# DankerMu/SHUD-up

Hardware: AMD Instinct MI355X
Metric: element-flux-updates/sec (RHS evals × NumEle) at 1/2/4/8 GPUs; %HBM roofline (higher is better)
Workload: dtype f64

## Files before the change

shud-up_amd/csrc/shud_dev.h:

```cpp
#pragma once
#include <hip/hip_runtime.h>
#include <stdint.h>

namespace shud {

constexpr int kWarnSlots = 64, kWarnStride = 16;
struct DevErr {
    uint32_t flags;
    int32_t first_index[8];
    unsigned long long n_warn;
    unsigned long long *warn;
};

struct DevMesh {
    int num_ele;
    const int *nabr, *eflags;
    const double *area, *z_surf, *z_bottom, *depression, *edge, *dist2nabor, *dist2edge, *avg_rough, *rough;
    const double *aq, *macD, *macKsatH, *vAreaF, *KsatH, *KsatV, *infKsatV, *hAreaF, *macKsatV;
    const double *ThetaS, *ThetaR, *Beta, *infD, *Sy, *RzD, *VegFrac, *ImpAF;
    const double *net_prep, *pot_evap, *pot_tran, *etp, *lai, *fu_surf, *fu_sub, *prcp;
    double *e_ic[2], *u_satn[2];
    const double *ugw_stale;
    const double *eybc, *eqbc, *rybc, *rqbc;
    const int *seg_off, *seg_riv;
    const double *seg_len, *seg_cwr;
    double *qseg_surf, *qseg_sub;
    const int *riv_down, *riv_bc;
    const double *riv_len, *riv_slope, *riv_d2down, *riv_avg_rough, *riv_depth, *riv_bw, *riv_bankslope;
    const double *riv_ksath, *riv_bedthick;
    const int *up_off, *up_idx;
    const int *rseg_off, *rseg_pos;
    DevErr *err;
};

enum ClassField {
    CF_macD, CF_macKsatH, CF_vAreaF, CF_KsatH, CF_KsatV, CF_infKsatV, CF_hAreaF, CF_macKsatV, CF_ThetaS,
    CF_ThetaR, CF_Beta, CF_infD, CF_Sy, CF_RzD, CF_VegFrac, CF_ImpAF, CF_depression, CF_rough,
    CF_NPRIMARY,
    CF_fcmr = CF_NPRIMARY,
    CF_dTh,
    CF_ex1, CF_ex2,
    CF_pj,
    CF_omh,
    CF_kmax,
    CF_ekA, CF_ekB,
    CF_r_fcmr, CF_r_dTh, CF_r_infD, CF_r_Sy,
    CF_COUNT
};
constexpr bool cf_stored(int f) { return f != CF_hAreaF && f != CF_macKsatV && f != CF_Beta && f != CF_ImpAF; }
constexpr int cf_pos(int f) {
    int q = 0;
    for (int g = 0; g < f; g++) q += cf_stored(g) ? 1 : 0;
    return cf_stored(f) ? q : -1;
}
template <int F> struct CfPos {
    static_assert(F >= 0 && F < CF_COUNT && cf_stored(F), "field not in the class record");
    static constexpr int v = cf_pos(F);
};
constexpr int CF_NSTORED = cf_pos(CF_COUNT - 1) + 1;
constexpr int CF_STRIDE = CF_NSTORED | 1;
constexpr double kCdivBmin = 0x1p-20, kCdivBmax = 0x1p20;
inline bool cdiv_divisor_ok(double b) {
    const double a = b < 0 ? -b : b;
    return b == 0. || !(a < 1e308) || (a >= kCdivBmin && a <= kCdivBmax);
}
constexpr int kLdsClassMax = 128;
constexpr int kShareTile = 256;
constexpr int kLspN = 5;
constexpr size_t kLspLdsMax = 23296;
constexpr size_t lsp_lds_bytes(int ntab) { return (size_t)(ntab + kLspN * kShareTile) * 8 + kShareTile * 4; }
#ifndef SHUD_PT_COMPACT
#define SHUD_PT_COMPACT 1
#endif
constexpr int kPowTabLogDoubles = SHUD_PT_COMPACT ? 2 * 128 + 64 : 4 * 256;
constexpr int kPowTabDoubles = kPowTabLogDoubles + 2 * 128;
constexpr int kLdsClassMaxBig = 560;
constexpr int kHybMax = 4;

struct DevPacked {
    const double *ctab;
    int ncls;
    int pt_off, ntab;
    const double *hv;
    int nh, hs;
    int hnb;
    signed char hslot1[CF_NPRIMARY];
    const double2 *zz;
    const int4 *meta;
    const double2 *ged;
    const double *area;
    int *seg_first;
    const double2 *sg_lc;
    const int *sg_r;
    const double2 *rrec;
    double2 *qseg2;
    double2 *s_np;
    double2 *s_tl;
    double2 *s_fu;
    double2 *cs[2];
    const double2 *rv;
    const int4 *rv_u;
    int riv_sb;
    double *qdown;
    int nqd;
    int qd_pm, qd_pm_fold;
    int lds_big;
};

struct DevDiag {
    double *qele_surf, *qele_sub, *qele_surf_tot, *qele_sub_tot, *q_infil, *q_exfil, *q_recharge;
    double *q_es, *q_eu, *q_eg, *q_tu, *q_tg, *q_eta, *e_ic, *u_satn, *i_beta, *eff_kh;
    double *qe2r_surf, *qe2r_sub, *qriv_down, *qriv_up, *qriv_surf, *qriv_sub;
    double *q_lake_surf, *q_lake_sub, *q_lake_rivin, *q_lake_evap, *q_lake_prcp, *lake_toparea;
};

struct DevLake {
    int nl;
    int y_off;
    const int *lake_of;
    double *bank_qs, *bank_qg;
    const int *bathy_off;
    const double *bathy_y, *bathy_a;
    const int *ele_off, *ele_idx;
    const int *bank_off, *bank_pos;
    const int *rin_off, *rin_idx;
};

struct YView {
    const double *y;
    const double *gele;
    const double *griv;
    int n_own, n_own_riv;
#ifdef __HIPCC__
    __device__ __forceinline__ double sf(int i) const { return i < n_own ? y[i] : gele[3 * (i - n_own)]; }
    __device__ __forceinline__ double us(int i) const { return i < n_own ? y[n_own + i] : gele[3 * (i - n_own) + 1]; }
    __device__ __forceinline__ double gw(int i) const { return i < n_own ? y[2 * n_own + i] : gele[3 * (i - n_own) + 2]; }
    __device__ __forceinline__ double riv(int r) const { return r < n_own_riv ? y[3 * n_own + r] : griv[r - n_own_riv]; }
    template <bool GH> __device__ __forceinline__ double sf_(int i) const { return GH ? sf(i) : y[i]; }
    template <bool GH> __device__ __forceinline__ double us_(int i) const { return GH ? us(i) : y[n_own + i]; }
    template <bool GH> __device__ __forceinline__ double gw_(int i) const { return GH ? gw(i) : y[2 * n_own + i]; }
    template <bool GH> __device__ __forceinline__ double riv_(int r) const { return GH ? riv(r) : y[3 * n_own + r]; }
#endif
};

void launch_element_kernel(const DevMesh &m, const YView &Y, double *dy, int n_compute, int cur, int cur_e,
                           int mode, bool open, bool diag, const DevDiag &dg, hipStream_t s);
bool launch_element_kernel_packed(const DevMesh &m, const DevPacked &p, const YView &Y, double *dy, int i0, int i1,
                                  int cur, int mode, bool open, bool diag, bool fu_unit, const DevDiag &dg,
                                  hipStream_t s, const DevLake *lake = nullptr, bool interior = false,
                                  bool with_qd = false);
// ... 23 lines not shown
```

shud-up_amd/csrc/shud_ele_packed.hip:

```cpp
#include <hip/hip_runtime.h>
#include <stdint.h>
#include <stdlib.h>

#include "shud_dev.h"
#include "shud_physics.h"

namespace shud {

typedef double v2d __attribute__((ext_vector_type(2)));
typedef int v4i __attribute__((ext_vector_type(4)));
template <class T>
__device__ __forceinline__ T ldnt(const T *p) { return __builtin_nontemporal_load(p); }
__device__ __forceinline__ double2 ldnt2(const double2 *p) {
    const v2d v = __builtin_nontemporal_load((const v2d *)p);
    return make_double2(v.x, v.y);
}
__device__ __forceinline__ int4 ldnt4(const int4 *p) {
    const v4i v = __builtin_nontemporal_load((const v4i *)p);
    return make_int4(v.x, v.y, v.z, v.w);
}
__device__ __forceinline__ void stnt2(double2 *p, double a, double b) {
    v2d v;
    v.x = a;
    v.y = b;
    __builtin_nontemporal_store(v, (v2d *)p);
}
template <class T>
__device__ __forceinline__ const T *at(const T *b, uint32_t off) { return (const T *)((const char *)b + off); }
template <class T>
__device__ __forceinline__ T *atw(T *b, uint32_t off) { return (T *)((char *)b + off); }

__device__ __forceinline__ bool nan_or_inf(double x) { return __builtin_isfpclass(x, 0x0003 | 0x0004 | 0x0200); }
__device__ __forceinline__ bool bad_nonneg(double x) {
    return __builtin_isfpclass(x, 0x0003 | 0x0004 | 0x0008 | 0x0010 | 0x0200);
}

__device__ __forceinline__ const double *riv_y_at(const YView &Y, int r) {
    return r < Y.n_own_riv ? Y.y + 3 * (size_t)Y.n_own + r : Y.griv + (r - Y.n_own_riv);
}

__device__ __forceinline__ int cf_ibc(int cf) { return (int)(int8_t)(cf & 0xff); }
__device__ __forceinline__ int cf_iss(int cf) { return (cf >> 8) & 3; }
__device__ __forceinline__ int cf_nseg(int cf) { return (cf >> 10) & 63; }
__device__ __forceinline__ int cf_class(int cf) { return (int)(((unsigned)cf >> 16) & 0x7fffu); }

template <int MODE>
__device__ __forceinline__ double ugw_pk(const DevMesh &m, double ygw_raw, int ibc, int j) {
    if (ibc == 0) return MODE == 0 ? ygw_raw : rmax(0.0, ygw_raw);
    if (ibc > 0) return m.eybc[ibc];
    return m.ugw_stale[j];
}

constexpr int LDS_CLS_MAX = kLdsClassMax;
constexpr int CF_LDS_STRIDE = CF_STRIDE;

constexpr int kEleWaves = 5;
constexpr int kEleWavesSh = 7;
constexpr bool kShareOn(bool lct, bool gh, bool lake, int hyb, bool diag) {
    return lct && !gh && !lake && hyb == 0 && !diag;
}
constexpr int kEleWavesOf(bool lct, int lspk, bool gh, bool lake, int hyb, bool diag, bool fu1, bool open) {
    return (kShareOn(lct, gh, lake, hyb, diag) && lspk) ? (fu1 ? kEleWavesSh : 6)
           : (kShareOn(lct, gh, lake, hyb, diag) && !open) ? 6 : kEleWaves;
}
constexpr int kEleBS = 256;
static_assert(kEleBS == kShareTile, "edge sharing pairs elements within one workgroup's tile");
static_assert(2 * kEleBS <= kPowTabDoubles, "edge-sharing slots fit the pow tables' LDS region");
constexpr uint64_t kShareVoid = 0x7ff0000000000001ull;
struct OwnRec {
    int4 mt;
    double2 zz, snp, stl, fu, csv;
    double ysf, yus, ygw;
    int sfl;
};
template <bool FU1, bool GH>
__device__ __forceinline__ OwnRec load_own(const DevPacked &p, const YView &Y, int i, int cur) {
    const int nown = Y.n_own;
    const uint32_t o16 = (uint32_t)i << 4, o8 = (uint32_t)i << 3;
    OwnRec o;
    o.mt = *at(p.meta, o16);
    o.zz = *at(p.zz, o16);
    o.ysf = GH ? Y.sf(i) : *at(Y.y, o8);
    o.yus = GH ? Y.us(i) : *at(Y.y + nown, o8);
    o.ygw = GH ? Y.gw(i) : *at(Y.y + 2 * (size_t)nown, o8);
    o.snp = ldnt2(at(p.s_np, o16));
    o.stl = ldnt2(at(p.s_tl, o16));
    if (FU1) { o.fu.x = 1.0; o.fu.y = 1.0; } else o.fu = ldnt2(at(p.s_fu, o16));
    o.csv = ldnt2(at(p.cs[cur], o16));
    o.sfl = *at(p.seg_first, (uint32_t)i << 2);
    return o;
}

constexpr int kTabBatch = 8;
template <int BS>
__device__ __forceinline__ void tab_issue(const DevPacked &p, double (&tv)[kTabBatch]) {
    const int nt2 = (p.ntab + 1) >> 1;
#pragma unroll
    for (int k = 0; k < kTabBatch / 2; k++) {
        const int t = (int)threadIdx.x + k * BS;
        const double2 v = t < nt2 ? ((const double2 *)p.ctab)[t] : make_double2(0., 0.);
        tv[2 * k] = v.x;
        tv[2 * k + 1] = v.y;
    }
}
template <int BS>
__device__ __forceinline__ void tab_store(const DevPacked &p, const double (&tv)[kTabBatch], double *lct) {
    const int nt2 = (p.ntab + 1) >> 1;
#pragma unroll
    for (int k = 0; k < kTabBatch / 2; k++) {
        const int t = (int)threadIdx.x + k * BS;
        if (t < nt2) ((double2 *)lct)[t] = make_double2(tv[2 * k], tv[2 * k + 1]);
    }
    for (int t = (int)threadIdx.x + kTabBatch / 2 * BS; t < nt2; t += BS)
        ((double2 *)lct)[t] = ((const double2 *)p.ctab)[t];
}
__device__ __forceinline__ int tile_of(int per8, int b) { return (b & 7) * per8 + (b >> 3); }
__device__ __forceinline__ int tile_of(int per8) { return tile_of(per8, (int)blockIdx.x); }

struct HaloWait;
template <int MODE, bool HALO>
__device__ __forceinline__ void qd_pre(const DevMesh &m, const DevPacked &p, const YView &Y, int r, int n_int,
                                       const HaloWait *hw);
__device__ __forceinline__ int qd_split(int b, int nb_q, int q0, int *e) {
    if (nb_q && b >= q0 && b < q0 + nb_q) return b - q0;
    *e = b < q0 ? b : b - nb_q;
    return -1;
}

template <int MODE, bool OPEN, bool DIAG, bool FU1, bool LCT, bool LAKE, bool GH, int HYB = 0, int LSP = 0, int BS = 256>
__device__ __forceinline__ void ele_body(const DevMesh &m, const DevPacked &p, const YView &Y, double *__restrict__ dy,
                                         int i, int cur, const DevDiag &dg, const DevLake &lk, const double *lct,
                                         const OwnRec &own);

template <int MODE, bool OPEN, bool DIAG, bool FU1, bool LCT, bool LAKE, bool GH, int HYB = 0, int LSPK = 0>
__global__ void __launch_bounds__(kEleBS, kEleWavesOf(LCT, LSPK, GH, LAKE, HYB, DIAG, FU1, OPEN))
shud_ele_kernel_packed(DevMesh m, DevPacked p, YView Y, double *__restrict__ dy, int i0, int n_compute, int cur,
                       DevDiag dg, DevLake lk, int per8, int nb_q, int q0) {
    extern __shared__ double lct[];
    int eb = (int)blockIdx.x;
    const int qb = qd_split((int)blockIdx.x, nb_q, q0, &eb);
    if (qb >= 0) {
        const int r = qb * kEleBS + (int)threadIdx.x;
        if (r < p.nqd) qd_pre<MODE, false>(m, p, Y, r, 0, nullptr);
        return;
    }
    const int i = i0 + tile_of(per8, eb) * kEleBS + (int)threadIdx.x;
    const bool act = i < n_compute;
    double tv[kTabBatch];
    if (LCT) tab_issue<kEleBS>(p, tv);
    OwnRec own;
    if (act) own = load_own<FU1, GH>(p, Y, i, cur);
    if (LCT) {
        tab_store<kEleBS>(p, tv, lct);
        __syncthreads();
    }
    if (act) ele_body<MODE, OPEN, DIAG, FU1, LCT, LAKE, GH, HYB, LCT ? LSPK : 0>(m, p, Y, dy, i, cur, dg, lk, lct, own);
}

template <int MODE, bool OPEN, bool DIAG, bool FU1, bool GH>
__global__ void __launch_bounds__(1024, 4)
shud_ele_kernel_packed_big(DevMesh m, DevPacked p, YView Y, double *__restrict__ dy, int i0, int n_compute, int cur,
                           DevDiag dg, DevLake lk, int per8) {
    extern __shared__ double lct[];
    const int i = i0 + tile_of(per8) * 1024 + (int)threadIdx.x;
    const bool act = i < n_compute;
    double tv[kTabBatch];
    tab_issue<1024>(p, tv);
    OwnRec own;
    if (act) own = load_own<FU1, GH>(p, Y, i, cur);
    tab_store<1024>(p, tv, lct);
    __syncthreads();
    if (act) ele_body<MODE, OPEN, DIAG, FU1, true, false, GH, 0, 0, 1024>(m, p, Y, dy, i, cur, dg, lk, lct, own);
}

__device__ __forceinline__ void halo_wait(const DevMesh &m, const HaloWait &hw, int i) {
    if (hw.epoch == 0) return;
    bool late = false;
    if (__lane_id() == 0) {
        const unsigned long long t0 = wall_clock64();
        while (__hip_atomic_load(hw.flag, __ATOMIC_RELAXED, __HIP_MEMORY_SCOPE_AGENT) < hw.epoch) {
            __builtin_amdgcn_s_sleep(8);
            if (wall_clock64() - t0 > hw.timeout) { late = true; break; }
        }
    }
    __builtin_amdgcn_fence(__ATOMIC_ACQUIRE, "agent");
    asm volatile("s_waitcnt vmcnt(0)" ::: "memory");
    report_w(m.err, late, 0x80u, 7, i);
}
template <int MODE, bool OPEN, bool FU1, int LSPK = 0>
__global__ void __launch_bounds__(256, kEleWaves)
shud_ele_kernel_packed_fold(DevMesh m, DevPacked p, YView Y, double *__restrict__ dy, int n_int, int n_all, int cur,
                            DevDiag dg, int per8, int nb_int, HaloWait hw, int nb_q, int q0) {
    extern __shared__ double lct[];
    const DevLake lk{};
    int b = (int)blockIdx.x;
    const int qb = qd_split((int)blockIdx.x, nb_q, q0, &b);
    if (qb >= 0) {
        const int r = qb * 256 + (int)threadIdx.x;
        qd_pre<MODE, true>(m, p, Y, r < p.nqd ? r : -1, n_int, &hw);
        return;
    }
    if (b < nb_int) {
        const int i = tile_of(per8, b) * 256 + (int)threadIdx.x;
        const bool act = i < n_int;
        double tv[kTabBatch];
        tab_issue<256>(p, tv);
        OwnRec own;
        if (act) own = load_own<FU1, false>(p, Y, i, cur);
        tab_store<256>(p, tv, lct);
        __syncthreads();
        if (act) ele_body<MODE, OPEN, false, FU1, true, false, false, 0, LSPK>(m, p, Y, dy, i, cur, dg, lk, lct, own);
        return;
    }
    const int i = n_int + (b - nb_int) * 256 + (int)threadIdx.x;
    const bool act = i < n_all;
    double tv[kTabBatch];
    tab_issue<256>(p, tv);
    halo_wait(m, hw, act ? i : n_int);
    OwnRec own;
    if (act) own = load_own<FU1, true>(p, Y, i, cur);
    tab_store<256>(p, tv, lct);
    __syncthreads();
    if (act) ele_body<MODE, OPEN, false, FU1, true, false, true, 0, LSPK>(m, p, Y, dy, i, cur, dg, lk, lct, own);
}
__global__ void shud_halo_flag_kernel(unsigned long long *flag, unsigned long long epoch) {
    if (threadIdx.x == 0) {
        __builtin_amdgcn_fence(__ATOMIC_RELEASE, "agent");
        asm volatile("s_waitcnt vmcnt(0)" ::: "memory");
        __hip_atomic_store(flag, epoch, __ATOMIC_RELAXED, __HIP_MEMORY_SCOPE_AGENT);
    }
}
__global__ void shud_spin_kernel(unsigned long long ticks) {
    if (threadIdx.x == 0) {
        const unsigned long long t0 = wall_clock64();
        while (wall_clock64() - t0 < ticks) __builtin_amdgcn_s_sleep(4);
    }
}
__global__ void shud_copy_f64_kernel(double *__restrict__ dst, const double *__restrict__ src, size_t n) {
    for (size_t k = blockIdx.x * (size_t)blockDim.x + threadIdx.x; k < n; k += (size_t)gridDim.x * blockDim.x)
        dst[k] = src[k];
}

__device__ __forceinline__ double hsel(const double (&v)[4], int k) {
    return k == 1 ? v[0] : k == 2 ? v[1] : k == 3 ? v[2] : v[3];
}
__device__ __forceinline__ void hload(const DevPacked &p, int i, double (&v)[4]) {
    v[1] = 0.; v[2] = 0.; v[3] = 0.;
    if (p.hs == 1) {
        v[0] = p.hv[i];
        return;
    }
    const double2 a = *(const double2 *)(p.hv + (size_t)p.hs * i);
    v[0] = a.x; v[1] = a.y;
    if (p.hs == 4) {
        const double2 b = *(const double2 *)(p.hv + (size_t)p.hs * i + 2);
        v[2] = b.x; v[3] = b.y;
    }
}

template <int MODE, bool OPEN, bool DIAG, bool FU1, bool LCT, bool LAKE, bool GH, int HYB, int LSP, int BS>
__device__ __forceinline__ void ele_body(const DevMesh &m, const DevPacked &p, const YView &Y, double *__restrict__ dy,
                                         int i, int cur, const DevDiag &dg, const DevLake &lk, const double *lct,
                                         const OwnRec &own) {
    const int NEl = m.num_ele;
    const int nown = Y.n_own;
    const uint32_t o16 = (uint32_t)i << 4, o8 = (uint32_t)i << 3;
    (void)o16;
    const int4 mt = own.mt;
    const double2 zz = own.zz;
    const double ysf_raw = own.ysf, yus_raw = own.yus, ygw_raw = own.ygw;
    const int cf = mt.w;
    const int cid = cf_class(cf), ibc = cf_ibc(cf);
    const bool is_lake = LAKE && cf < 0;
    const double2 snp = own.snp, stl = own.stl;
    const double etp = stl.y;
    const double2 fu = own.fu;
    const double2 csv = own.csv;
#define REPORT(c, bit, slot, cnt) report_w(m.err, (c), (bit), (slot), i, (cnt))
#define REPORT_ET(c, bit) (rep |= (c) ? (uint32_t)(bit) : 0u)
#define CL(f) (LCT ? lct[cid * CF_LDS_STRIDE + CfPos<CF_##f>::v] : p.ctab[cid * CF_STRIDE + CfPos<CF_##f>::v])
#define CDIV(a, F) cdiv(a, CL(F), CL(r_##F))
    double hvo[4] = {0., 0., 0., 0.};
    if (HYB == 1) hvo[0] = p.hv[i];
    else if (HYB == 2) hload(p, i, hvo);
#define CLH(f) ((HYB && p.hslot1[CF_##f]) ? (HYB == 1 ? hvo[0] : hsel(hvo, p.hslot1[CF_##f])) : CL(f))
#define CDIV_SY(a) ((HYB && p.hslot1[CF_Sy]) ? (a) / (HYB == 1 ? hvo[0] : hsel(hvo, p.hslot1[CF_Sy])) : CDIV(a, Sy))

    double usf = ysf_raw, uus = yus_raw;
    if (MODE == 1) { usf = (usf >= 0.) ? usf : 0.; uus = (uus >= 0.) ? uus : 0.; }
    const double ugw = ugw_pk<MODE>(m, ygw_raw, ibc, i);
    const double zs = zz.x, zb = zz.y;
    const double aq = zs - zb;

    double ekh, deficit, theta, satn, satkr;
    if (is_lake) {
        ekh = CLH(KsatH); deficit = 0.; satn = 1.; theta = CL(ThetaS); satkr = 1.0;
    } else {
        ekh = eff_kh(ugw, aq, CLH(macD), CLH(macKsatH), CLH(vAreaF), CLH(KsatH));
        REPORT(ekh < 0. || ekh > 1e9, 0x02u, 1, false);
        deficit = aq - ugw;
        const double ThS = CL(ThetaS), ThR = CL(ThetaR);
        if (deficit <= 0.) { deficit = 0.; satn = 1.; theta = ThS; }
        else { theta = uus / deficit * ThS; satn = CDIV(theta - ThR, dTh); }
        if (satn > 0.99) { satn = 1.0; satkr = 1.0; theta = ThS; }
        else if (satn <= K_ZERO) { satn = 0.; satkr = 0.; theta = ThR; }
        else {
// ... 42 lines not shown
            report_w(m.err, rep & 0x10u, 0x10u, 4, i, true);
        }
        if (DIAG) { dg.q_es[i] = Es; dg.q_eu[i] = Eu; dg.q_eg[i] = Eg; dg.q_tu[i] = Tu; dg.q_tg[i] = Tg;
                    dg.q_eta[i] = eta; dg.i_beta[i] = ibeta; }
    }
    stnt2(atw(p.cs[cur ^ 1], o16), satn, eic);

    double qi = 0., qex = 0., qr = 0.;
    if (!is_lake) {
        const double kmax = CL(kmax);
        const double av = usf + snp.x;
        if (ugw + uus > aq || deficit < uus) {
            qex = fabs(ugw + uus - aq) / aq * kmax;
        } else if (av > 0. && deficit > infD) {
            const double grad = 1. + CDIV(av, infD);
            double ek;
            if (av > kmax) ek = CL(ekA) + CL(ekB) * satn;
            else if (av > infK) ek = satkr * infK * CL(omh) + CL(ekB) * satn;
            else ek = satkr * infK * CL(omh);
            qi = rmin(av, rmax(0., grad * ek));
        }
        const double KV = CLH(KsatV);
        if (!(ugw > aq - infD && uus < deficit)) {
            double grad = 0.;
            if (theta > ThR && !(uus <= K_EPSILON)) {
                grad = CDIV(theta - ThR, fcmr);
                grad = rmax(grad, 0.);
            }
            if (!(infK <= 0. || KV <= 0.)) {
                const double ku = infK * satkr;
                qr = grad * ((ku * KV) * (deficit + ugw) / (deficit * KV + ugw * ku));
            }
        }
    }
    const double q_infil = qi * fu_surf, q_exfil = qex * fu_surf;
    const double q_rech = is_lake ? 0. : qr * fu_sub;

    const double dsf_head = snp.x - q_infil + q_exfil;
    const double dgw_head = q_rech - q_exfil;
    typedef __attribute__((address_space(3))) volatile double lds_vd;
    lds_vd *lsp = LSP ? (lds_vd *)(lct + p.ntab) + threadIdx.x : nullptr;
    typedef __attribute__((address_space(3))) volatile int lds_vi;
    lds_vi *lspi = LSP ? (lds_vi *)(lct + p.ntab + kLspN * kEleBS) + threadIdx.x : nullptr;
    if (LSP) {
        lsp[0] = Es; lsp[kEleBS] = Eg; lsp[2 * kEleBS] = Tg; lsp[3 * kEleBS] = dsf_head; lsp[4 * kEleBS] = dgw_head;
        lspi[0] = cf;
    }
    if (i < nown) __builtin_nontemporal_store(is_lake ? 0. : CDIV_SY(q_infil - q_rech - Eu - Tu), atw(dy + nown, o8));

    const double dep = CLH(depression), rgh = CLH(rough);
    double qe2r_surf = 0., qe2r_sub = 0.;
    if (nseg) {
        const double isf_seg = rmax(0., usf - q_infil + q_exfil);
        for (int k = sfirst, k1 = k + nseg; k < k1; k++) {
            const uint32_t k16 = (uint32_t)k << 4;
            const double2 lc = *at(p.sg_lc, k16);
            const int rr = *at(p.sg_r, (uint32_t)k << 2);
            const double2 dk = p.rrec[2 * (size_t)rr], rx = p.rrec[2 * (size_t)rr + 1];
            const int rbc = __builtin_bit_cast(int2, rx.y).x;
            const double bt = rx.x;
            double yr = GH ? Y.riv(rr) : *at(Y.y + 3 * (size_t)nown, (uint32_t)rr << 3);
            if (MODE == 1) yr = (yr >= 0.) ? yr : 0.;
            if (rbc > 0) yr = m.rybc[rbc];
            const double rdep = dk.x, L = lc.x;
            const double qs = weir_jtoi(zs, isf_seg, zs - rdep, yr, zs + 0.0, lc.y, L, dep);
            const double qg = r2e_gw(yr, zs - rdep, ugw, zb, ekh, dk.y, L, bt) * fu_sub;
            *atw(p.qseg2, k16) = make_double2(qs, qg);
            qe2r_surf += -qs;
            qe2r_sub += -qg;
        }
    }
    if (DIAG) {
        dg.q_infil[i] = q_infil; dg.q_exfil[i] = q_exfil; dg.q_recharge[i] = q_rech;
        dg.e_ic[i] = eic; dg.u_satn[i] = satn; dg.eff_kh[i] = ekh;
        dg.qe2r_surf[i] = qe2r_surf; dg.qe2r_sub[i] = qe2r_sub;
    }
    if (i >= nown) return;

    bool nan_q = false;
    const double isf = usf < 0. ? 0. : usf;
    const double area = ldnt(at(p.area, o8));
    const int n_edges = is_lake ? 0 : 3;
    constexpr bool SH = kShareOn(LCT, GH, LAKE, HYB, DIAG) && LSP != 0 && BS == kEleBS;
    auto edge = [&](int j, double &qsf, double &q, uint32_t &sh) __attribute__((always_inline)) {
        const int nb = j == 0 ? mt.x : j == 1 ? mt.y : mt.z;
        const int nc = nb >= 0 ? nb : i;
        const uint32_t n16 = (uint32_t)nc << 4, n8 = (uint32_t)nc << 3;
        const double2 g = ldnt2(at(p.ged, o16 + (uint32_t)j * ((uint32_t)NEl << 4)));
        const double2 nzz = *at(p.zz, n16);
        const int ncf = *at((const int *)p.meta + 3, n16);
        const double nsf_raw = GH ? Y.sf(nc) : *at(Y.y, n8);
        const double ngw_raw = GH ? Y.gw(nc) : *at(Y.y + 2 * (size_t)nown, n8);
        const double B = g.x, d2n = g.y;
        const Recip R2 = recip_nr(d2n);
        qsf = 0.; q = 0.; sh = 0u;
        const double dep_e = SH ? (double)((lds_vd *)lct)[cid * CF_LDS_STRIDE + CfPos<CF_depression>::v] : dep;
        const double rgh_e = SH ? (double)((lds_vd *)lct)[cid * CF_LDS_STRIDE + CfPos<CF_rough>::v] : rgh;
        const int cn = cf_class(ncf);
#define CN(f) (LCT ? lct[cn * CF_LDS_STRIDE + CfPos<CF_##f>::v] : p.ctab[cn * CF_STRIDE + CfPos<CF_##f>::v])
        double hvn[4] = {0., 0., 0., 0.};
        if (HYB == 1 && p.hnb) hvn[0] = p.hv[nc];
        else if (HYB == 2 && p.hnb) hload(p, nc, hvn);
#define CNH(f) ((HYB && p.hslot1[CF_##f]) ? (HYB == 1 ? hvn[0] : hsel(hvn, p.hslot1[CF_##f])) : CN(f))
        if (LAKE && nb >= 0 && ncf < 0) {
            const int l = lk.lake_of[nb];
            const double zl = lk.bathy_y[lk.bathy_off[l]];
            const double yl = Y.y[lk.y_off + l];
            const double nsf = yl < 0. ? 0. : yl;
            qsf = weir_jtoi(zl, nsf, zs, isf, zs, 0.6, B, 0.01);
            const double dhg = (ugw + zb) - (yl + zl);
            if (dhg > 0. && ugw <= 0.02) q = 0.;
            else if (dhg < 0. && yl <= 0.02) q = 0.;
            else {
                const double ymg = (rmax(ugw, 0.) + rmax(yl, 0.)) * .5;
                const double grad = div_nr(dhg, R2);
                const double kmean = 0.5 * (ekh + CNH(KsatH));
                q = kmean * grad * ymg * B;
            }
            lk.bank_qs[(size_t)j * NEl + i] = qsf;
            lk.bank_qg[(size_t)j * NEl + i] = q;
        } else if (nb >= 0) {
            double nsf = nsf_raw;
            if (MODE == 1) nsf = (nsf >= 0.) ? nsf : 0.;
            nsf = nsf < 0. ? 0. : nsf;
            const double zsn = nzz.x;
            const double dh = (isf + zs) - (nsf + zsn);
            [[maybe_unused]] const bool dh_nz = dh != 0., dh_ok = dh == dh;
            double ym = ((isf + zs) > (nsf + zsn)) ? ((isf > dep_e) ? isf : 0.) : ((nsf > dep_e) ? nsf : 0.);
            ym = rmin(ym, K_MAXYSURF);
            bool mu = false;
            if (ym > 0.) {
                const double s = div_nr(dh, R2);
                if (s > 0 && isf <= 0) qsf = 0.;
                else if (s < 0 && nsf <= 0) qsf = 0.;
                else { qsf = manning(ym * B, 0.5 * (rgh_e + CNH(rough)), ym, s); mu = true; }
            }
            const double ugn = ugw_pk<MODE>(m, ngw_raw, cf_ibc(ncf), nb);
            const double zbn = nzz.y;
            const double dhg = (ugw + zb) - (ugn + zbn);
            [[maybe_unused]] const bool dhg_nz = dhg != 0., dhg_ok = dhg == dhg;
            bool zq = true;
            if (dhg > 0. && ugw <= 0.02) q = 0.;
            else if (dhg < 0. && ugn <= 0.02) q = 0.;
            else {
                const double ekn = eff_kh(ugn, zsn - zbn, CNH(macD), CNH(macKsatH), CNH(vAreaF), CNH(KsatH));
                const double ymg = (rmax(ugw, 0.) + rmax(ugn, 0.)) * .5;
                const double grad = div_nr(dhg, R2);
                const double kmean = 0.5 * (ekh + ekn);
                q = kmean * grad * ymg * B;
                zq = false;
            }
            if constexpr (SH) sh = (mu && dh_nz ? 1u : 0u) | (!zq && dhg_nz ? 2u : 0u) | (dh_ok && dhg_ok ? 4u : 0u);
        } else if (OPEN) {
            const double d2e = m.dist2edge[j * NEl + i];
            if (isf > dep_e) {
                const double s = isf / d2e * 0.5;
                if (s > 0.) qsf = sqrt(s) * cbrt(isf * isf * isf * isf * isf) * B / rgh_e;
            }
            if (ugw > dep_e * 10.) {
                const double grad = ugw / d2e * 0.5;
                if (grad > 0.) q = ekh * grad;
            }
        }
#undef CN
#undef CNH
    };
    double sumsurf = qe2r_surf, sumsub = qe2r_sub;
    auto add = [&](int j, double qsf, double q) __attribute__((always_inline)) {
        const double qsb = q * fu_sub;
        if (MODE == 0) nan_q |= nan_or_inf(qsf) || nan_or_inf(qsb);
        sumsurf += qsf;
        sumsub += qsb;
        if (DIAG) { dg.qele_surf[j * NEl + i] = qsf; dg.qele_sub[j * NEl + i] = qsb; }
    };
    if constexpr (!SH) {
#pragma unroll 1
        for (int j = 0; j < n_edges; j++) {
            double qsf, q;
            uint32_t sh;
            edge(j, qsf, q, sh);
            add(j, qsf, q);
        }
    } else {
        lds_vd *xq = (lds_vd *)(lct + p.pt_off);
        const int tid = (int)threadIdx.x;
        uint32_t st = ((uint32_t)sfl >> 26) & 15u;
        const int jr0 = (int)((st >> 2) & 3u) - 1;
        const int j1 = (st & 3u) ? (int)(st & 3u) - 1 : (jr0 == 0 ? 1 : 0);
        st |= (uint32_t)(j1 + 1) << 12;
        __syncthreads();
        {
            double qsf, q;
            uint32_t sh;
            edge(j1, qsf, q, sh);
            if (!(st & 3u)) sh = 4u;
            xq[tid] = (sh & 4u) ? ((sh & 1u) ? -qsf : qsf) : __builtin_bit_cast(double, kShareVoid);
            xq[kEleBS + tid] = (sh & 2u) ? -q : q;
            st |= (sh & 3u) << 4 | ((sh & 4u) ? 1u << (8 + j1) : 0u);
        }
        __syncthreads();
        auto rthread = [&]() __attribute__((always_inline)) {
            const int jr = (int)((st >> 2) & 3u) - 1;
            return (jr == 0 ? mt.x : jr == 1 ? mt.y : mt.z) - (i - tid);
        };
        if (st & 12u) {
            const int rt = rthread();
            if (rt >= 0 && rt < kEleBS && __builtin_bit_cast(uint64_t, (double)xq[rt]) != kShareVoid)
                st |= 1u << (8 + ((st >> 2) & 3u) - 1);
        }
        auto take = [&](int mm) __attribute__((always_inline)) {
            double qsf, q;
            if (mm == (int)((st >> 12) & 3u) - 1) {
                const double a = xq[tid], b = xq[kEleBS + tid];
                qsf = (st & 16u) ? -a : a;
                q = (st & 32u) ? -b : b;
            } else {
                const int rt = rthread();
                qsf = xq[rt];
                q = xq[kEleBS + rt];
            }
            add(mm, qsf, q);
        };
#pragma unroll 1
        for (uint32_t om = 7u & ~(st >> 8); om; om &= om - 1) {
            const int j = __builtin_ctz(om);
            double qsf, q;
            uint32_t sh;
            edge(j, qsf, q, sh);
#pragma unroll
            for (int mm = 0; mm < 2; mm++)
                if ((st >> (8 + mm) & 1u) && mm < j) { take(mm); st &= ~(1u << (8 + mm)); }
            add(j, qsf, q);
        }
#pragma unroll
        for (int mm = 0; mm < 3; mm++)
            if (st >> (8 + mm) & 1u) take(mm);
    }
    if (DIAG && is_lake)
        for (int j = 0; j < 3; j++) { dg.qele_surf[j * NEl + i] = 0.; dg.qele_sub[j * NEl + i] = 0.; }
    if (MODE == 0) REPORT(nan_q, 0x01u, 0, false);

    double dsf, dgw;
    const Recip RA = recip_nr(area);
    if (LSP) {
        const double es = lsp[0], eg = lsp[kEleBS], tg = lsp[2 * kEleBS], dsh = lsp[3 * kEleBS], dgh = lsp[4 * kEleBS];
        dsf = dsh - div_nr(sumsurf, RA) - es;
        dgw = dgh - div_nr(sumsub, RA) - eg - tg;
    } else {
        dsf = dsf_head - div_nr(sumsurf, RA) - Es;
        dgw = dgw_head - div_nr(sumsub, RA) - Eg - Tg;
    }
    const int cf_t = LSP ? lspi[0] : cf;
    const int ibc_t = LSP ? cf_ibc(cf_t) : ibc, iss_t = LSP ? cf_iss(cf_t) : iss;
    if (ibc_t > 0) dgw = 0;
    else if (ibc_t < 0) dgw += div_nr(m.eqbc[-ibc_t], RA);
    if (iss_t == 1) dsf += zero_over(area);
    else if (iss_t == 2) dgw += zero_over(area);
    dgw = CDIV_SY(dgw);
    if (LSP ? (LAKE && cf_t < 0) : is_lake) { dsf = 0.; dgw = 0.; }
#undef CL
#undef CLH
#undef CDIV_SY
    __builtin_nontemporal_store(dsf, atw(dy, o8));
    __builtin_nontemporal_store(dgw, atw(dy + 2 * (size_t)nown, o8));
    if (DIAG) { dg.qele_surf_tot[i] = sumsurf; dg.qele_sub_tot[i] = sumsub; }
#undef REPORT
#undef REPORT_ET
}

struct RivP {
    double w0, bs, len, slope, d2d, n, depth;
    int down, bc;
};
__device__ __forceinline__ int2 rv_ib(double x) { return __builtin_bit_cast(int2, x); }
__device__ __forceinline__ RivP riv_load(const DevPacked &p, int r) {
    const double2 *q = p.rv + 4 * (size_t)r;
    const double2 a = q[0], b = q[1], c = q[2], d = q[3];
    const int2 ib = rv_ib(d.y);
    RivP o;
    o.w0 = a.x; o.bs = a.y; o.len = b.x; o.slope = b.y; o.d2d = c.x; o.n = c.y; o.depth = d.x;
    o.down = ib.x; o.bc = ib.y;
    return o;
}
__device__ __forceinline__ RivGeom riv_geom_p(const RivP &q, double y) { return riv_geom(q.w0, q.bs, q.len, y); }
template <int MODE>
__device__ __forceinline__ double riv_stage_p(const DevMesh &m, const YView &Y, int r, int bc, double *yg) {
    double yr = Y.riv(r);
    if (MODE == 1) yr = (yr >= 0.) ? yr : 0.;
    *yg = yr;
    return bc > 0 ? m.rybc[bc] : yr;
}
__device__ __forceinline__ double riv_down_p(const RivP &q, double uq, const RivGeom &g, double ud, double ddepth,
                                             double dslope) {
    if (q.down >= 0) {
        const double smean = (q.slope + dslope) * 0.5;
        const double s = ((uq - q.depth) - (ud - ddepth)) / q.d2d + smean;
        const double R = (g.csperem <= K_ZERO) ? 0. : (g.csarea / g.csperem);
        return manning(g.csarea, q.n, R, s);
    } else if (q.down >= -3) {
        const double s = q.slope + uq * 2. / q.len;
        const double R = (g.csperem <= 0.) ? 0. : (g.csarea / g.csperem);
        return manning(g.csarea, q.n, R, s);
    }
    return g.csarea * sqrt(K_GRAV * uq) * 60.;
}
__device__ __forceinline__ double riv_down_outlet(const RivP &q, double uq, const RivGeom &g) {
    return riv_down_p(q, uq, g, 0., 0., 0.);
}
template <int MODE, bool HALO>
__device__ __forceinline__ void qd_pre(const DevMesh &m, const DevPacked &p, const YView &Y, int r, int n_int,
                                       const HaloWait *hw) {
    const int rr = r < 0 ? 0 : r;
    const RivP q = riv_load(p, rr);
    const int d = q.down >= 0 ? q.down : rr;
    if (HALO) {
        const bool ghost = r >= 0 && (r >= Y.n_own_riv || d >= Y.n_own_riv);
        if (__builtin_amdgcn_ballot_w64(ghost)) halo_wait(m, *hw, n_int);
    }
    if (r < 0) return;
// ... 343 lines not shown
```

shud-up_amd/csrc/shud_rhs.cpp:

```cpp
#include <hip/hip_runtime.h>
#include <rccl/rccl.h>

#include <algorithm>
#include <climits>
#include <cmath>
#include <cstdarg>
#include <cstdio>
#include <cstdlib>
#include <cstring>
#include <numeric>
#include <string>
#include <unordered_map>
#include <vector>

#include "shud_handle.h"
#define SHUD_PT_HOST_TABLES
#include "shud_pow_tab.h"

using namespace shud;

namespace {
thread_local std::string g_last_error;
}

// ... 452 lines not shown
        if (!build_classes(hmask)) return 0;
    } else if (!fits) {
        return 0;
    }
    const int ncls = (int)table.size();
    const int l2 = env_knob("SHUD_RHS_L2_CLASS", -1, 0, 1);
    const int l2_max = l2 == 1 ? 32768 : l2 == 0 ? kLdsClassMax : kLdsClassMaxBig;
    if (ncls > l2_max) return 0;
    h->dp.lds_big = l2 == 1 ? 0 : 1;
    std::vector<double> ctab((size_t)CF_STRIDE * ncls, 0.0);
    for (int c = 0; c < ncls; c++) {
        std::vector<double> &t = table[c];
        t.resize(CF_COUNT);
        t[CF_fcmr] = t[CF_ThetaS] * 0.75 - t[CF_ThetaR];
        t[CF_dTh] = t[CF_ThetaS] - t[CF_ThetaR];
        t[CF_ex1] = t[CF_Beta] / (t[CF_Beta] - 1.);
        t[CF_ex2] = (t[CF_Beta] - 1.) / t[CF_Beta];
        if (!(t[CF_Beta] > 1.) || !std::isfinite(t[CF_ex1]) || !std::isfinite(t[CF_ex2])) return 0;
        t[CF_pj] = 1. - t[CF_ImpAF];
        t[CF_omh] = 1. - t[CF_hAreaF];
        t[CF_kmax] = t[CF_infKsatV] * (1. - t[CF_hAreaF]) + t[CF_macKsatV] * t[CF_hAreaF];
        t[CF_ekA] = t[CF_infKsatV] * (1. - t[CF_hAreaF]);
        t[CF_ekB] = t[CF_hAreaF] * t[CF_macKsatV];
        if (!cdiv_divisor_ok(t[CF_fcmr]) || !cdiv_divisor_ok(t[CF_dTh]) || !cdiv_divisor_ok(t[CF_infD]) ||
            !cdiv_divisor_ok(t[CF_Sy]))
            return 0;
        t[CF_r_fcmr] = 1. / t[CF_fcmr];
        t[CF_r_dTh] = 1. / t[CF_dTh];
        t[CF_r_infD] = 1. / t[CF_infD];
        t[CF_r_Sy] = 1. / t[CF_Sy];
        for (int f = 0; f < CF_COUNT; f++)
            if (cf_stored(f)) ctab[(size_t)c * CF_STRIDE + cf_pos(f)] = t[f];
    }
    const int pt_off = ((int)ctab.size() + 1) & ~1;
    ctab.resize((size_t)pt_off + kPowTabDoubles, 0.0);
#if SHUD_PT_COMPACT
    static_assert(sizeof shud_pt_clogtab == 8 * kPowTabLogDoubles, "pow_tab");
    memcpy(&ctab[pt_off], shud_pt_clogtab, sizeof shud_pt_clogtab);
#else
    static_assert(kPowTabLogDoubles == 4 * SHUD_PT_LOG_N && sizeof shud_pt_logtab == 8 * kPowTabLogDoubles, "pow_tab");
    memcpy(&ctab[pt_off], shud_pt_logtab, sizeof shud_pt_logtab);
#endif
    static_assert(kPowTabDoubles == kPowTabLogDoubles + 2 * SHUD_PT_EXP_N, "pow_tab table size");
    memcpy(&ctab[pt_off + kPowTabLogDoubles], shud_pt_exptab, sizeof shud_pt_exptab);
    std::vector<double2> zz(NE), ged(3 * (size_t)NE);
    std::vector<int4> meta(NE);
    std::vector<int> sfirst(NE);
    for (int i = 0; i < NE; i++) {
        zz[i] = make_double2(m->z_surf[i], m->z_bottom[i]);
        const int nseg = seg_off[i + 1] - seg_off[i];
        const int ibc = (int8_t)(eflags[i] & 0xff);
        const bool lake_ele = m->ilake && m->ilake[i] > 0 && h->lakeon;
        const unsigned cf = (unsigned)(ibc & 0xff) | ((unsigned)((eflags[i] >> 16) & 3) << 8) |
                            ((unsigned)nseg << 10) | ((unsigned)cls[i] << 16) | (lake_ele ? 0x80000000u : 0u);
        meta[i] = make_int4(m->nabr[i], m->nabr[(size_t)NE + i], m->nabr[2 * (size_t)NE + i], (int)cf);
        for (int j = 0; j < 3; j++)
            ged[(size_t)j * NE + i] = make_double2(m->edge[(size_t)j * NE + i], m->dist2nabor[(size_t)j * NE + i]);
        sfirst[i] = seg_off[i];
    }
    const int lim = h->n_int > 0 ? h->n_int : (h->n_own == NE ? NE : 0);
    if (lim > 1 && !hmask && !h->lakeon && lsp_lds_bytes((int)ctab.size()) <= kLspLdsMax && m->num_seg < (1 << 26) &&
        env_knob("SHUD_RHS_SHARE", 1, 0, 1)) {
        std::vector<signed char> pub(NE, -1), rcv(NE, -1);
        auto lake_of = [&](int e) { return m->ilake && m->ilake[e] > 0 && h->lakeon; };
        for (int i = 0; i < lim; i++) {
            for (int k = 0; k < 3 && rcv[i] < 0; k++) {
                const int v = m->nabr[(size_t)k * NE + i];
                if (v < 0 || v >= lim || v == i || (v / kShareTile) != (i / kShareTile) || pub[v] >= 0) continue;
                int kk = -1, hits = 0;
                for (int q = 0; q < 3; q++)
                    if (m->nabr[(size_t)q * NE + v] == i) { kk = q; hits++; }
                if (hits != 1 || pub[i] == k) continue;
                const size_t a = (size_t)k * NE + i, b = (size_t)kk * NE + v;
                const double ar = m->avg_rough[a];
                if (memcmp(&m->edge[a], &m->edge[b], 8) || memcmp(&m->dist2nabor[a], &m->dist2nabor[b], 8) ||
                    (m->depression && memcmp(&m->depression[i], &m->depression[v], 8)) ||
                    memcmp(&ar, &m->avg_rough[b], 8) ||
                    !(ar > 0. && std::isfinite(ar)) || lake_of(i) || lake_of(v))
                    continue;
                pub[v] = (signed char)kk;
                rcv[i] = (signed char)k;
            }
        }
        for (int i = 0; i < NE; i++) sfirst[i] |= ((pub[i] + 1) << 26) | ((rcv[i] + 1) << 28);
        h->n_shared = (int)std::count_if(rcv.begin(), rcv.end(), [](signed char r) { return r >= 0; });
    }
    int rc;
    DevPacked &P = h->dp;
    double *ctab_d, *area_d; double2 *zz_d, *ged_d; int4 *meta_d; int *sf_d;
    if ((rc = h->upload(&ctab_d, ctab.data(), ctab.size()))) return rc;
    if ((rc = h->upload(&zz_d, zz.data(), NE))) return rc;
    if ((rc = h->upload(&meta_d, meta.data(), NE))) return rc;
    if ((rc = h->upload(&ged_d, ged.data(), ged.size()))) return rc;
    if ((rc = h->upload(&area_d, m->area, NE))) return rc;
    if ((rc = h->upload(&sf_d, sfirst.data(), NE))) return rc;
    P.ctab = ctab_d; P.ncls = ncls; P.pt_off = pt_off; P.ntab = (int)ctab.size(); P.zz = zz_d;
    if (hmask) {
        int nh = 0;
        for (int f = 0; f < CF_NPRIMARY; f++)
            if (hmask >> f & 1) P.hslot1[f] = (signed char)++nh;
        const int hs = nh == 1 ? 1 : nh == 2 ? 2 : 4;
        std::vector<double> hv((size_t)hs * NE, 0.0), rr(CF_NPRIMARY);
        for (int i = 0; i < NE; i++) {
            prim(i, rr);
            for (int f = 0; f < CF_NPRIMARY; f++)
                if (P.hslot1[f]) hv[(size_t)hs * i + P.hslot1[f] - 1] = rr[f];
        }
        double *hv_d;
        if ((rc = h->upload(&hv_d, hv.data(), hv.size()))) return rc;
        P.hv = hv_d; P.nh = nh; P.hs = hs;
        P.hnb = (hmask & (1u << CF_macD | 1u << CF_macKsatH | 1u << CF_vAreaF | 1u << CF_KsatH | 1u << CF_rough)) != 0;
    } P.meta = meta_d; P.ged = ged_d; P.area = area_d;
    P.seg_first = sf_d;
    {
        const int NSg = m->num_seg, NRl = m->num_riv;
        std::vector<double2> lc(NSg), rr(2 * (size_t)NRl);
        std::vector<int> sr(NSg);
        for (int k = 0; k < NSg; k++) {
            const int s = h->seg_perm[k];
            lc[k] = make_double2(m->seg_length[s], m->seg_cwr[s]);
            sr[k] = m->seg_riv[s];
        }
        for (int r = 0; r < NRl; r++) {
            const int32_t two[2] = {m->riv_bc ? m->riv_bc[r] : 0, 0};
            double bits;
            memcpy(&bits, two, sizeof bits);
            rr[2 * (size_t)r] = make_double2(m->riv_depth[r], m->riv_ksath[r]);
            rr[2 * (size_t)r + 1] = make_double2(m->riv_bedthick[r], bits);
        }
        double2 *lc_d, *rr_d; int *sr_d;
        if ((rc = h->upload(&lc_d, lc.data(), NSg))) return rc;
        if ((rc = h->upload(&sr_d, sr.data(), NSg))) return rc;
        if ((rc = h->upload(&rr_d, rr.data(), rr.size()))) return rc;
        P.sg_lc = lc_d; P.sg_r = sr_d; P.rrec = rr_d;
        if ((rc = h->upload(&P.qseg2, (const double2 *)nullptr, NSg))) return rc;
    }
    if ((rc = h->upload(&P.s_np, (const double2 *)nullptr, NE))) return rc;
    if ((rc = h->upload(&P.s_tl, (const double2 *)nullptr, NE))) return rc;
    if ((rc = h->upload(&P.cs[0], (const double2 *)nullptr, NE))) return rc;
    if ((rc = h->upload(&P.cs[1], (const double2 *)nullptr, NE))) return rc;
    std::vector<double2> ones(NE, make_double2(1.0, 1.0));
    if ((rc = h->upload(&P.s_fu, ones.data(), NE))) return rc;

    const int NS = m->num_seg, NR = m->num_riv;
    std::vector<int> rorder(NS);
    std::iota(rorder.begin(), rorder.end(), 0);
    std::stable_sort(rorder.begin(), rorder.end(), [&](int a, int b) { return m->seg_riv[a] < m->seg_riv[b]; });
    std::vector<int> rstart(NR, 0), rcnt(NR, 0);
    for (int q = NS - 1; q >= 0; q--) rstart[m->seg_riv[rorder[q]]] = q;
    for (int s = 0; s < NS; s++) rcnt[m->seg_riv[s]]++;
    std::vector<double2> rv(4 * (size_t)NR);
    std::vector<int4> ru(NR);
    const int nor = h->n_own_riv;
    for (int r = 0; r < NR; r++) {
        const int dn = (h->lakeon && m->riv_down[r] <= -4) ? -3 : m->riv_down[r];
        const int bc = m->riv_bc ? m->riv_bc[r] : 0;
        double ib;
        const int32_t two[2] = {dn, bc};
        memcpy(&ib, two, sizeof ib);
        rv[4 * (size_t)r + 0] = make_double2(m->riv_bottom_width[r], m->riv_bankslope[r]);
        rv[4 * (size_t)r + 1] = make_double2(m->riv_length[r], m->riv_bed_slope[r]);
        rv[4 * (size_t)r + 2] = make_double2(m->riv_dist2down[r], m->riv_avg_rough[r]);
        rv[4 * (size_t)r + 3] = make_double2(m->riv_depth[r], ib);
        int4 u = make_int4(rstart[r], rcnt[r], 0, 0);
        if (r < nor) {
            const int n = up_off[r + 1] - up_off[r];
            u = n <= 2 ? make_int4(rstart[r], rcnt[r] | (n << 16), n > 0 ? up_idx[up_off[r]] : 0,
// ... 711 lines not shown
```

Measured before the change: 18.38 billion.

## Reorder element edges on host so shared edge is slot 0 and receive slot 2

Host setup now permutes each element's neighbour and edge-geometry records so that the published shared edge is always stored in slot 0 and the received edge in slot 2. It encodes the permutation in spare flag bits so the kernel can map results back to their original edge order. In the shared-edge path this replaces the data-dependent edge loop and bit-state bookkeeping with a fixed sequence: compute edge 0, publish it to LDS, compute edge 1, then compute edge 2 only if it was not received. That removes divergent control flow and cuts VGPR pressure, which allows a different launch-bounds occupancy setting. It also adds an early exit for fully idle waves and a byte flag array in LDS, at the cost of extra host preprocessing, which must stay consistent with the dist2edge and diagnostic indexing.

```diff
diff --git a/shud-up_amd/csrc/shud_dev.h b/shud-up_amd/csrc/shud_dev.h
--- a/shud-up_amd/csrc/shud_dev.h
+++ b/shud-up_amd/csrc/shud_dev.h
@@ -66,6 +66,23 @@
 }
 constexpr int kLdsClassMax = 128;
 constexpr int kShareTile = 256;
+constexpr int kEvoShift = 26;
+constexpr unsigned kEvoPub0 = 1u << 29, kEvoRcv2 = 1u << 30;
+inline unsigned evo_encode(const int e[3]) {
+    const int s0 = e[0] == 0 ? 0 : e[1] == 0 ? 1 : 2;
+    const int lo = s0 == 0 ? 1 : 0;
+    return (unsigned)s0 | (e[lo] == 2 ? 4u : 0u);
+}
+__host__ __device__ inline int evo_stored(unsigned bits, int j) {
+    const int s0 = (int)(bits & 3u), lo = s0 == 0 ? 1 : 0, hi = s0 == 2 ? 1 : 2;
+    const bool sw = (bits & 4u) != 0;
+    return j == 0 ? s0 : (j == 1) != sw ? lo : hi;
+}
+__host__ __device__ inline int evo_ref(unsigned bits, int s) {
+    const int s0 = (int)(bits & 3u), lo = s0 == 0 ? 1 : 0;
+    const bool sw = (bits & 4u) != 0;
+    return s == s0 ? 0 : (s == lo) != sw ? 1 : 2;
+}
 constexpr int kLspN = 5;
 constexpr size_t kLspLdsMax = 23296;
 constexpr size_t lsp_lds_bytes(int ntab) { return (size_t)(ntab + kLspN * kShareTile) * 8 + kShareTile * 4; }
diff --git a/shud-up_amd/csrc/shud_ele_packed.hip b/shud-up_amd/csrc/shud_ele_packed.hip
--- a/shud-up_amd/csrc/shud_ele_packed.hip
+++ b/shud-up_amd/csrc/shud_ele_packed.hip
@@ -65,8 +65,7 @@
 }
 constexpr int kEleBS = 256;
 static_assert(kEleBS == kShareTile, "edge sharing pairs elements within one workgroup's tile");
-static_assert(2 * kEleBS <= kPowTabDoubles, "edge-sharing slots fit the pow tables' LDS region");
-constexpr uint64_t kShareVoid = 0x7ff0000000000001ull;
+static_assert(2 * kEleBS * 8 + kEleBS <= kPowTabDoubles * 8, "edge-sharing slots fit the pow tables' LDS region");
 struct OwnRec {
     int4 mt;
     double2 zz, snp, stl, fu, csv;
@@ -116,6 +115,12 @@
 }
 __device__ __forceinline__ int tile_of(int per8, int b) { return (b & 7) * per8 + (b >> 3); }
 __device__ __forceinline__ int tile_of(int per8) { return tile_of(per8, (int)blockIdx.x); }
+__device__ __forceinline__ bool share_idle_wave(bool act) {
+    if (__builtin_amdgcn_ballot_w64(act)) return false;
+    __syncthreads();
+    __syncthreads();
+    return true;
+}
 
 struct HaloWait;
 template <int MODE, bool HALO>
@@ -154,6 +159,7 @@
         tab_store<kEleBS>(p, tv, lct);
         __syncthreads();
     }
+    if (kShareOn(LCT, GH, LAKE, HYB, DIAG) && LSPK != 0 && share_idle_wave(act)) return;
     if (act) ele_body<MODE, OPEN, DIAG, FU1, LCT, LAKE, GH, HYB, LCT ? LSPK : 0>(m, p, Y, dy, i, cur, dg, lk, lct, own);
 }
 
@@ -188,7 +194,7 @@
     report_w(m.err, late, 0x80u, 7, i);
 }
 template <int MODE, bool OPEN, bool FU1, int LSPK = 0>
-__global__ void __launch_bounds__(256, kEleWaves)
+__global__ void __launch_bounds__(256, (LSPK && FU1 && !OPEN) ? kEleWavesSh : kEleWaves)
 shud_ele_kernel_packed_fold(DevMesh m, DevPacked p, YView Y, double *__restrict__ dy, int n_int, int n_all, int cur,
                             DevDiag dg, int per8, int nb_int, HaloWait hw, int nb_q, int q0) {
     extern __shared__ double lct[];
@@ -209,6 +215,7 @@
         if (act) own = load_own<FU1, false>(p, Y, i, cur);
         tab_store<256>(p, tv, lct);
         __syncthreads();
+        if (LSPK != 0 && share_idle_wave(act)) return;
         if (act) ele_body<MODE, OPEN, false, FU1, true, false, false, 0, LSPK>(m, p, Y, dy, i, cur, dg, lk, lct, own);
         return;
     }
@@ -221,7 +228,7 @@
     if (act) own = load_own<FU1, true>(p, Y, i, cur);
     tab_store<256>(p, tv, lct);
     __syncthreads();
-    if (act) ele_body<MODE, OPEN, false, FU1, true, false, true, 0, LSPK>(m, p, Y, dy, i, cur, dg, lk, lct, own);
+    if (act) ele_body<MODE, OPEN, false, FU1, true, false, true, 0, LSPK ? 2 : 0>(m, p, Y, dy, i, cur, dg, lk, lct, own);
 }
 __global__ void shud_halo_flag_kernel(unsigned long long *flag, unsigned long long epoch) {
     if (threadIdx.x == 0) {
@@ -430,11 +437,13 @@
     const double area = ldnt(at(p.area, o8));
     const int n_edges = is_lake ? 0 : 3;
     constexpr bool SH = kShareOn(LCT, GH, LAKE, HYB, DIAG) && LSP != 0 && BS == kEleBS;
-    auto edge = [&](int j, double &qsf, double &q, uint32_t &sh) __attribute__((always_inline)) {
-        const int nb = j == 0 ? mt.x : j == 1 ? mt.y : mt.z;
+    constexpr bool DEC = !SH && LCT && !LAKE && HYB == 0 && BS == kEleBS && (LSP == 1 || DIAG);
+    [[maybe_unused]] const uint32_t evo = (uint32_t)sfl >> kEvoShift;
+    auto edge = [&](int s, int j, double &qsf, double &q, uint32_t &sh) __attribute__((always_inline)) {
+        const int nb = s == 0 ? mt.x : s == 1 ? mt.y : mt.z;
         const int nc = nb >= 0 ? nb : i;
         const uint32_t n16 = (uint32_t)nc << 4, n8 = (uint32_t)nc << 3;
-        const double2 g = ldnt2(at(p.ged, o16 + (uint32_t)j * ((uint32_t)NEl << 4)));
+        const double2 g = ldnt2(at(p.ged, o16 + (uint32_t)s * ((uint32_t)NEl << 4)));
         const double2 nzz = *at(p.zz, n16);
         const int ncf = *at((const int *)p.meta + 3, n16);
         const double nsf_raw = GH ? Y.sf(nc) : *at(Y.y, n8);
@@ -500,7 +509,7 @@
             }
             if constexpr (SH) sh = (mu && dh_nz ? 1u : 0u) | (!zq && dhg_nz ? 2u : 0u) | (dh_ok && dhg_ok ? 4u : 0u);
         } else if (OPEN) {
-            const double d2e = m.dist2edge[j * NEl + i];
+            const double d2e = m.dist2edge[(SH ? evo_ref(evo, s) : j) * NEl + i];
             if (isf > dep_e) {
                 const double s = isf / d2e * 0.5;
                 if (s > 0.) qsf = sqrt(s) * cbrt(isf * isf * isf * isf * isf) * B / rgh_e;
@@ -526,63 +535,56 @@
         for (int j = 0; j < n_edges; j++) {
             double qsf, q;
             uint32_t sh;
-            edge(j, qsf, q, sh);
+            edge(DEC ? evo_stored(evo, j) : j, j, qsf, q, sh);
             add(j, qsf, q);
         }
     } else {
+        typedef __attribute__((address_space(3))) volatile unsigned char lds_vb;
         lds_vd *xq = (lds_vd *)(lct + p.pt_off);
+        lds_vb *xf = (lds_vb *)(lct + p.pt_off + 2 * kEleBS);
         const int tid = (int)threadIdx.x;
-        uint32_t st = ((uint32_t)sfl >> 26) & 15u;
-        const int jr0 = (int)((st >> 2) & 3u) - 1;
-        const int j1 = (st & 3u) ? (int)(st & 3u) - 1 : (jr0 == 0 ? 1 : 0);
-        st |= (uint32_t)(j1 + 1) << 12;
         __syncthreads();
         {
             double qsf, q;
             uint32_t sh;
-            edge(j1, qsf, q, sh);
-            if (!(st & 3u)) sh = 4u;
-            xq[tid] = (sh & 4u) ? ((sh & 1u) ? -qsf : qsf) : __builtin_bit_cast(double, kShareVoid);
-            xq[kEleBS + tid] = (sh & 2u) ? -q : q;
-            st |= (sh & 3u) << 4 | ((sh & 4u) ? 1u << (8 + j1) : 0u);
+            edge(0, 0, qsf, q, sh);
+            xq[tid] = qsf;
+            xq[kEleBS + tid] = q;
+            xf[tid] = (unsigned char)sh;
         }
         __syncthreads();
-        auto rthread = [&]() __attribute__((always_inline)) {
-            const int jr = (int)((st >> 2) & 3u) - 1;
-            return (jr == 0 ? mt.x : jr == 1 ? mt.y : mt.z) - (i - tid);
-        };
-        if (st & 12u) {
-            const int rt = rthread();
-            if (rt >= 0 && rt < kEleBS && __builtin_bit_cast(uint64_t, (double)xq[rt]) != kShareVoid)
-                st |= 1u << (8 + ((st >> 2) & 3u) - 1);
-        }
-        auto take = [&](int mm) __attribute__((always_inline)) {
-            double qsf, q;
-            if (mm == (int)((st >> 12) & 3u) - 1) {
-                const double a = xq[tid], b = xq[kEleBS + tid];
-                qsf = (st & 16u) ? -a : a;
-                q = (st & 32u) ? -b : b;
-            } else {
-                const int rt = rthread();
-                qsf = xq[rt];
-                q = xq[kEleBS + rt];
+        double a1, b1, a2 = 0., b2 = 0.;
+        {
+            uint32_t sh;
+            edge(1, 1, a1, b1, sh);
+        }
+        bool own2 = true;
+        if (evo & (kEvoRcv2 >> kEvoShift)) {
+            const int rt = mt.z - (i - tid);
+            if (rt >= 0 && rt < kEleBS) {
+                const uint32_t f = xf[rt];
+                if (f & 4u) {
+                    const double a = xq[rt], b = xq[kEleBS + rt];
+                    a2 = (f & 1u) ? -a : a;
+                    b2 = (f & 2u) ? -b : b;
+                    own2 = false;
+                }
             }
-            add(mm, qsf, q);
-        };
-#pragma unroll 1
-        for (uint32_t om = 7u & ~(st >> 8); om; om &= om - 1) {
-            const int j = __builtin_ctz(om);
-            double qsf, q;
-            uint32_t sh;
-            edge(j, qsf, q, sh);
-#pragma unroll
-            for (int mm = 0; mm < 2; mm++)
-                if ((st >> (8 + mm) & 1u) && mm < j) { take(mm); st &= ~(1u << (8 + mm)); }
-            add(j, qsf, q);
-        }
-#pragma unroll
-        for (int mm = 0; mm < 3; mm++)
-            if (st >> (8 + mm) & 1u) take(mm);
+        }
+        if (__builtin_amdgcn_ballot_w64(own2)) {
+            if (own2) {
+                uint32_t sh;
+                edge(2, 2, a2, b2, sh);
+            }
+        }
+        const double a0 = xq[tid], b0 = xq[kEleBS + tid];
+        const uint32_t s0 = evo & 3u;
+        const bool sw = (evo & 4u) != 0;
+        const double la = s0 == 0 ? a1 : a0, lb = s0 == 0 ? b1 : b0;
+        const double ha = s0 == 2 ? a1 : a2, hb = s0 == 2 ? b1 : b2;
+        add(0, s0 == 0 ? a0 : s0 == 1 ? a1 : a2, s0 == 0 ? b0 : s0 == 1 ? b1 : b2);
+        add(1, sw ? ha : la, sw ? hb : lb);
+        add(2, sw ? la : ha, sw ? lb : hb);
     }
     if (DIAG && is_lake)
         for (int j = 0; j < 3; j++) { dg.qele_surf[j * NEl + i] = 0.; dg.qele_sub[j * NEl + i] = 0.; }
diff --git a/shud-up_amd/csrc/shud_rhs.cpp b/shud-up_amd/csrc/shud_rhs.cpp
--- a/shud-up_amd/csrc/shud_rhs.cpp
+++ b/shud-up_amd/csrc/shud_rhs.cpp
@@ -558,7 +558,19 @@
                 rcv[i] = (signed char)k;
             }
         }
-        for (int i = 0; i < NE; i++) sfirst[i] |= ((pub[i] + 1) << 26) | ((rcv[i] + 1) << 28);
+        for (int i = 0; i < lim; i++) {
+            const int p = pub[i], r = rcv[i];
+            int e[3];
+            e[0] = p >= 0 ? p : (r == 0 ? 1 : 0);
+            e[2] = r >= 0 ? r : (e[0] == 2 ? 1 : 2);
+            e[1] = 3 - e[0] - e[2];
+            const int nb[3] = {meta[i].x, meta[i].y, meta[i].z};
+            meta[i].x = nb[e[0]]; meta[i].y = nb[e[1]]; meta[i].z = nb[e[2]];
+            for (int s = 0; s < 3; s++)
+                ged[(size_t)s * NE + i] =
+                    make_double2(m->edge[(size_t)e[s] * NE + i], m->dist2nabor[(size_t)e[s] * NE + i]);
+            sfirst[i] |= (int)((evo_encode(e) << kEvoShift) | (p >= 0 ? kEvoPub0 : 0u) | (r >= 0 ? kEvoRcv2 : 0u));
+        }
         h->n_shared = (int)std::count_if(rcv.begin(), rcv.end(), [](signed char r) { return r >= 0; });
     }
     int rc;
```

Result: faster. 19.32 billion (median of 6 runs) (+5.1%).
